# renmengye/rec-attend-public

Measured on AMD Instinct MI355X. Metric: instance-timesteps/sec, full_model forward 512x512 T=16 (whole job; pipelined throughput: 8 batches in flight per GPU, fill and drain of the pipeline inside the timed region; config.lone_batch_* = one sync-bracketed forward), higher is better.
Workload: dtype f32; 1 GPU; cfg2: CVPPP-arch full_model eval forward, 512x512, T=16, B=8 per GPU, y_out+s_out; arch=cvppp, H=512, W=512, T=16, batch_per_gpu=8, global_batch=8, parallelism=batch-sharded x1, no collective, ranks_in_communicator=1, hip_graph=True, tile_tickets=False, batches_in_flight=8, pipeline_slots=4, batches_per_launch=2, input=resident in HBM, output=left in HBM

## Files before the change

include/recattend.h:

```cpp
#ifndef RECATTEND_H_
#define RECATTEND_H_

#include <stddef.h>
#include <stdint.h>

#ifdef __cplusplus
extern "C" {
#endif

#define RA_E_INVALID (-1)
#define RA_E_SHAPE (-2)
#define RA_E_WORKSPACE (-3)
#define RA_E_HUNG_BFS (-12)
#define RA_E_HUNG_PATH (-13)
#define RA_E_HUNG_FLOW (-14)
#define RA_E_HUNG_EQUALIZE (-15)

#define RA_ABI_VERSION 113
int ra_version(void);
const char *ra_last_error_string(void);

int ra_debug_poison_lds(void *stream);
int ra_debug_park_xcd(int xcd, int n_wg, int lds_bytes, int millis, int *resident, void *stream);

#define RA_PLAN_INTS 24
#define RA_PLAN_FAMILY 0
#define RA_PLAN_FORM 1
#define RA_PLAN_CK 2
#define RA_PLAN_NC 3
#define RA_PLAN_WN 4
#define RA_PLAN_GX 5
#define RA_PLAN_GY 6
#define RA_PLAN_KF 7
#define RA_PLAN_TILE_H 8
#define RA_PLAN_TILE_W 9
#define RA_PLAN_TILES_X 10
#define RA_PLAN_TILES_Y 11
#define RA_PLAN_NTILES 12
#define RA_PLAN_GRID 13
#define RA_PLAN_TILES_MIN 14
#define RA_PLAN_TILES_MAX 15
#define RA_PLAN_XCD_MAP 16
#define RA_PLAN_TICKETS 17
#define RA_PLAN_CMID 18
#define RA_PLAN_SLICES 19
#define RA_PLAN_POOL 20
#define RA_PLAN_FAMILY_K1 1
#define RA_PLAN_FAMILY_CONV8 2
#define RA_PLAN_FAMILY_PAIR 3
#define RA_PLAN_FAMILY_SPLIT 4
#define RA_PLAN_FAMILY_WINO 5
#define RA_PLAN_FAMILY_PAIR_WINO 6
#define RA_PLAN_FORM_SWAP 1
#define RA_PLAN_FORM_SUBPIXEL 2
#define RA_PLAN_FORM_BF16 4
#define RA_PLAN_FORM_MOMENTS 8
#define RA_PLAN_FORM_KXK 16
#define RA_PLAN_FORM_PERSIST 32
#define RA_PLAN_FORM_NPACKED 64
#define RA_PLAN_FORM_CACHED 128
#define RA_PLAN_FORM_SPLIT 256
#define RA_PLAN_FORM_PLANE 512
int ra_conv3x3_plan(int C0, int C1, int B, int Hs, int Ws, int upsample, int KF, int Cout, int pool, int has_plane,
                    int bf16_operands, int moments, int store_flags, int *plan);
int ra_conv_pair_plan(int Cin, int B, int Hs, int Ws, int upsampleA, int CoutA, int CoutB, int poolB, int has_plane,
                      int cache_form, int *plan);
int ra_conv_split_plan(int B, int H, int W, int Cin, int Cout, int pool, int has_plane, int *plan);
int ra_conv_wino_plan(int B, int H, int W, int Cin, int Cout, int pool, int *plan);
int ra_conv_pair_wino_plan(int B, int H, int W, int *plan);

int ra_hungarian_f32(const float *weights, int B, int N, int M, float *matching,
                     float *cover_x, float *cover_y);

size_t ra_hungarian_dev_workspace_bytes(int B, int N, int M);
int ra_hungarian_f32_dev(const float *weights, int B, int N, int M, float *matching,
                         float *cover_x, float *cover_y, int *status_dev, void *ws,
                         size_t ws_bytes, void *stream);

#define RA_CONV_TRANSPOSED 1

int ra_conv_cout_padded(int Cout);
size_t ra_conv_packed_floats(int Cin, int Cout);
int ra_conv_pack_weights(const float *w, int Cin_w, int Cout, int Cin, const int *chan_map,
                         int flags, float *out);
size_t ra_conv_packed_floats_k(int KF, int Cin, int Cout);
int ra_conv_pack_weights_k(const float *w, int KF, int Cin_w, int Cout, int Cin, const int *chan_map, int flags,
                           float *out);
int ra_conv_fold_bn(const float *bias, const float *beta, const float *gamma, const float *mean,
                    const float *var, int Cout, float eps, float *scale, float *shift);

int ra_conv3x3_f32(const float *src0, int C0, const float *src1, int C1, int B, int Hs, int Ws,
                   int upsample, const float *wpacked, const float *scale, const float *shift,
                   int Cout, int relu, int pool, const float *plane, int plane_chan, float *y,
                   void *stream);

int ra_convkxk_f32(const float *src0, int C0, const float *src1, int C1, int B, int Hs, int Ws, int upsample,
                   const float *wpacked, int KF, const float *scale, const float *shift, int Cout, int relu, int pool,
                   const float *plane, int plane_chan, float *y, void *stream);

int ra_conv_wide_supported(int Cin, int Cout);
size_t ra_conv_wide_packed_floats(int Cin, int Cout);
int ra_conv_wide_pack_weights(const float *w, int Cin_w, int Cout, int Cin, const int *chan_map, int flags, float *out);
int ra_conv3x3_wide_f32(const float *src0, int C0, const float *src1, int C1, int B, int Hs, int Ws, int upsample,
                        const float *wpacked, const float *scale, const float *shift, int Cout, int relu, int pool,
                        float *y, void *stream);

int ra_fg_head_f32(const float *logits, size_t npix, int nsc, int no, int quantise, float *y_out, float *d_out,
                   const float *x, int D, float *packed, int Cp, float *canvas_plane, void *stream);

int ra_conv3x3_bf16ops_f32(const float *src0, int C0, const float *src1, int C1, int B, int Hs, int Ws,
                           int upsample, const float *wpacked, const float *scale, const float *shift,
                           int Cout, int relu, int pool, const float *plane, int plane_chan, float *y,
                           void *stream);

int ra_conv3x3_bf16_f32(const void *src0, int C0, const void *src1, int C1, int B, int Hs, int Ws, int upsample,
                        const float *wpacked, const float *scale, const float *shift, int Cout, int relu, int pool, void *y,
                        float *part, size_t part_floats, int *nparts, int store_flags, void *stream);
int ra_bn_act_pool_bf16_f32(const void *u, const float *mean, const float *var, const float *gamma, const float *beta, float eps,
                            int relu, int pool, int B, int H, int W, int C, void *y, int flags, void *stream);
int ra_bn_act_pool_bwd_acc_bf16_f32(const void *u, const void *dy, const float *mean, const float *var, const float *gamma,
                                    const float *beta, float eps, int relu, int pool, int B, int H, int W, int C, float *ws,
                                    size_t ws_floats, float *dgamma, float *dbeta, void *du, float *acc_gamma, float *acc_beta,
                                    int flags, void *stream);
int ra_bn_act_pool_bwd_grouped_bf16_f32(const void *u, const void *dy, const void *const *tabs, int G, float eps, int relu, int pool,
                                        int B, int H, int W, int C, float *ws, size_t ws_floats, float *dgamma, float *dbeta,
                                        void *du, int flags, void *stream);
int ra_conv3x3_wgrad_acc_bf16_f32(const void *x, int Cin, int B, int Hs, int Ws, int upsample, const void *du, int Cout, float *ws,
                                  size_t ws_floats, const int *chan_map, int cin_w, int transposed, float *gw, float *gb, int fmt,
                                  void *stream);

size_t ra_conv3x3_moments_part_floats(int Cout);
int ra_conv3x3_moments_f32(const float *src0, int C0, const float *src1, int C1, int B, int Hs, int Ws,
                           int upsample, const float *wpacked, const float *scale, const float *shift,
                           int Cout, int relu, int bf16_operands, float *y, float *part, size_t part_floats,
                           int *nparts, void *stream);
int ra_bn_moments_from_partials_f32(const float *part, int nparts, int C, float *mean, float *var, void *stream);

int ra_conv_pair_supported(int Cin, int CoutA, int CoutB);
int ra_conv_pair_f32(const float *src, int Cin, int B, int Hs, int Ws, int upsampleA,
                     const float *wpA, const float *scaleA, const float *shiftA, int CoutA, int reluA,
                     const float *wpB, const float *scaleB, const float *shiftB, int CoutB, int reluB,
                     int poolB, const float *plane, int plane_chan, float *y, void *stream);

int ra_conv_split_supported(int Cin, int Cout, int pool, int H, int W);
size_t ra_conv_split_packed_halfs(int Cin, int Cout);
int ra_conv_split_pack_weights(const float *w, int Cin, int Cout, unsigned short *out);
int ra_conv_split_pack_weights_dev(const float *w, int Cin, int Cout, int transposed, unsigned short *out, void *stream);
int ra_conv_split_f32(const float *x, int B, int H, int W, int Cin, const unsigned short *wpacked, const float *scale,
                      const float *shift, int Cout, int relu, int pool, float *y, void *stream);
int ra_conv_split_plane_f32(const float *x, int B, int H, int W, int Cin, const float *plane, int plane_chan,
                            const unsigned short *wpacked, const float *scale, const float *shift, int Cout, int relu, int pool,
                            float *y, void *stream);

int ra_conv_wino_supported(int Cin, int Cout, int pool, int H, int W);
size_t ra_conv_wino_packed_floats(int Cin, int Cout);
int ra_conv_wino_pack_weights(const float *w, int Cin, int Cout, float *out);
int ra_conv_wino_f32(const float *x, int B, int H, int W, int Cin, const float *wpacked,
                     const float *scale, const float *shift, int Cout, int relu, int pool, float *y,
                     void *stream);

int ra_conv_pair_wino_supported(int Cin, int CoutA, int CoutB, int poolB, int H, int W);
int ra_conv_pair_wino_f32(const float *x, int B, int H, int W, const float *wpA, const float *scaleA,
                          const float *shiftA, int reluA, const float *wpB_wino, const float *scaleB,
                          const float *shiftB, int reluB, float *y, void *stream);

int ra_conv_first_cache_supported(int Cin, int CoutA, int CoutB, int poolB, int H, int W);
size_t ra_conv_first_cache_floats(int B, int H, int W);
int ra_conv_first_cache_f32(const float *src, int B, int H, int W, const float *wpA, int CoutA,
                            int plane_chan, float *cache, void *stream);
int ra_conv_pair_fill_cache_f32(const float *src, const float *plane, int plane_chan, int B, int H,
                                int W, const float *wpA, const float *scaleA, const float *shiftA,
                                int reluA, const float *wpB, const float *scaleB,
                                const float *shiftB, int CoutB, int reluB, float *cache, float *y,
                                void *stream);
int ra_conv_pair_fill_cache_rider_f32(const float *src, const float *plane, int plane_chan, int B, int H, int W,
                                      const float *wpA, const float *scaleA, const float *shiftA, int reluA,
                                      const float *wpB, const float *scaleB, const float *shiftB, int CoutB,
                                      int reluB, float *cache, float *y, float *fill_dst, size_t fill_floats,
                                      float fill_value, void *stream);
int ra_conv_pair_cached_f32(const float *cache, const float *plane, int plane_chan, int B, int H,
                            int W, const float *wpA, const float *scaleA, const float *shiftA,
                            int reluA, const float *wpB, const float *scaleB, const float *shiftB,
                            int CoutB, int reluB, float *y, void *stream);

typedef struct ra_ctrl_desc {
  int G;
  int Cf;
  int hid;
  int iters;
  int n_gmlp;
  int n_cmlp;
  int mlp_dim;
  int H, W;
  int Fh, Fw;
  int squash;
  int fixed_var;
  int dynamic_var;
  int fixed_gamma;
} ra_ctrl_desc;

size_t ra_ctrl_packed_floats(const ra_ctrl_desc *d);
int ra_ctrl_pack_weights(const ra_ctrl_desc *d, const float *const *lstm_w,
                         const float *const *gmlp_w, const float *const *cmlp_w, float *out);

#define RA_ATTN_STRIDE 16
int ra_controller_f32(const ra_ctrl_desc *d, const float *feat , const float *wpacked,
                      int B, float *h_last , float *ctrl_out ,
                      float *glimpse_maps ,
                      float *attn , void *stream);

int ra_ctrl_split_supported(const ra_ctrl_desc *d);
size_t ra_ctrl_split_packed_floats(const ra_ctrl_desc *d);
size_t ra_ctrl_split_workspace_bytes(const ra_ctrl_desc *d, int B);
int ra_ctrl_split_pack_weights(const ra_ctrl_desc *d, const float *const *lstm_w,
                               const float *const *gmlp_w, const float *const *cmlp_w, float *out);
int ra_controller_split_f32(const ra_ctrl_desc *d, const float *feat, const float *wpacked, int B,
                            float *h_last, float *ctrl_out, float *glimpse_maps, float *attn,
                            void *ws, size_t ws_bytes, int *status_dev, void *stream);
int ra_ctrl_batch_group_images(const ra_ctrl_desc *d, int B);
int ra_ctrl_batch_supported(const ra_ctrl_desc *d);
// ... 272 lines not shown
```

rec-attend-public_amd/csrc/ra_conv_split.hip:

```cpp
#include <cstring>

#include "ra_common.h"

namespace ra {
namespace csplit {

typedef float f32x4 __attribute__((ext_vector_type(4)));
typedef float f32x2 __attribute__((ext_vector_type(2)));
typedef short s16x8 __attribute__((ext_vector_type(8)));
typedef __bf16 bf16x8 __attribute__((ext_vector_type(8)));
typedef unsigned u32x2 __attribute__((ext_vector_type(2)));
typedef unsigned u32x4 __attribute__((ext_vector_type(4)));

constexpr int TW = 16;
constexpr int WSX = TW + 2;
constexpr int WSP = 20;
constexpr int tile_rows(int cin) { return (cin >= 64 || cin == 24) ? 8 : 16; }
constexpr int rec_stride(int cin) { return cin == 24 ? 80 : 2 * cin + 16; }
constexpr int k_blocks(int cin) { return (9 * (cin / 8) + 3) / 4; }

struct SArgs {
  const float *x;
  const unsigned short *wp;
  const float *scale, *shift;
  float *y;
  int B, H, W, Cout, relu;
  int bytes_x, bytes_y;
  unsigned *tickets;
  const float *plane;
  int plane_chan, bytes_p;
};

template <int CIN, int NB>
struct Geo {
  static constexpr int TH = tile_rows(CIN), WSY = TH + 2;
  static constexpr int GPW = TH / 4;
  static constexpr int NBLK = k_blocks(CIN);
  static constexpr int RS = rec_stride(CIN);
  static constexpr int PLANE = WSY * WSP * RS;
  static constexpr int WBYTES = NBLK * 3 * NB * 1024;
  static constexpr int LDS = 3 * PLANE + WBYTES;
  static constexpr int OCC = 2 * (LDS + 64) <= 160 * 1024 ? 2 : 1;
};

__device__ inline unsigned pk_bf16(float lo, float hi) {
  typedef __bf16 bf16x2c __attribute__((ext_vector_type(2)));
  return __builtin_bit_cast(unsigned, __builtin_convertvector(f32x2{lo, hi}, bf16x2c));
}
__device__ inline void split3_pair(float a, float b, unsigned &H, unsigned &M, unsigned &L) {
  H = pk_bf16(a, b);
  float ra = a - __builtin_bit_cast(float, H << 16), rb = b - __builtin_bit_cast(float, H & 0xffff0000u);
  M = pk_bf16(ra, rb);
  ra -= __builtin_bit_cast(float, M << 16);
  rb -= __builtin_bit_cast(float, M & 0xffff0000u);
  L = pk_bf16(ra, rb);
}

#ifdef RA_PROBES
__device__ long long *ra_probes_buf;
#define RA_PS_DECL long long ps_acc[8] = {0, 0, 0, 0, 0, 0, 0, 0}, ps_t = (long long)__builtin_readcyclecounter(), ps_t0 = (long long)wall_clock64()
#define RA_PS_AT(k)                                                \
  do {                                                             \
    __builtin_amdgcn_sched_barrier(0);                             \
    const long long n_ = (long long)__builtin_readcyclecounter();  \
    ps_acc[k] += n_ - ps_t;                                        \
    ps_t = n_;                                                     \
    __builtin_amdgcn_sched_barrier(0);                             \
  } while (0)
#define RA_PS_END                                                                    \
  do {                                                                               \
    if (threadIdx.x == 0 && ra_probes_buf) {                                         \
      ps_acc[7] = (long long)wall_clock64() - ps_t0;                                 \
      for (int k_ = 0; k_ < 8; ++k_) ra_probes_buf[((size_t)blockIdx.y * gridDim.x + blockIdx.x) * 8 + k_] = ps_acc[k_]; \
    }                                                                                \
  } while (0)
#else
#define RA_PS_DECL
#define RA_PS_AT(k)
#define RA_PS_END
#endif
template <int CIN, int POOL, int NB, bool PL = false>
__global__ __launch_bounds__(256, (Geo<CIN, NB>::OCC)) void conv_split_kernel(const SArgs a, int tiles_x, int tiles_y, int ntiles) {
  using G = Geo<CIN, NB>;
  constexpr int RS = G::RS, PLANE = G::PLANE, NBLK = G::NBLK, C4 = CIN / 4, TH = G::TH, WSY = G::WSY, GPW = G::GPW;
  constexpr int NITEMS = WSY * WSX * C4, NIT = (NITEMS + 255) / 256;
  extern __shared__ __attribute__((aligned(16))) unsigned char lds[];
  unsigned char *tin = lds;
  unsigned char *wl = lds + 3 * PLANE;
  const int tid = threadIdx.x, lane = tid & 63;
  RA_PS_DECL;
  __shared__ unsigned tk_sh[2];
  TicketWalk tk;
  const bool dyn = a.tickets != nullptr;
  if (dyn) tk.issue(a.tickets + blockIdx.y * kTicketSlotWords, ntiles);
  const int wave = __builtin_amdgcn_readfirstlane(tid >> 6);
  const int m = lane & 15, kb = lane >> 4;
  const int slice = blockIdx.y;

  const int qy = m >> 3, qx = (m >> 2) & 1, dy = (m >> 1) & 1, dx = m & 1;
  const int lane_pix = ((2 * qy + dy) * WSP + 2 * qx + dx) * RS;
  int toff[NBLK];
#pragma unroll
  for (int b = 0; b < NBLK; ++b) {
    constexpr int OPT = CIN / 8;
    const int o = 4 * b + kb;
    int tap = o / OPT;
    const int ch = 8 * (o % OPT);
    tap = tap < 9 ? tap : 8;
    toff[b] = ((tap / 3) * WSP + tap % 3) * RS + 2 * ch;
  }
  const int woff = (kb * 16 + m) * 16;
  float sc[NB], sh[NB];
#pragma unroll
  for (int nb = 0; nb < NB; ++nb) {
    sc[nb] = a.scale[16 * (NB * slice + nb) + m];
    sh[nb] = a.shift[16 * (NB * slice + nb) + m];
  }
  const float lo = a.relu ? 0.f : -__builtin_inff();
  const int Ho = a.H / POOL, Wo = a.W / POOL;
  const __amdgpu_buffer_rsrc_t rx = __builtin_amdgcn_make_buffer_rsrc(const_cast<float *>(a.x), 0, a.bytes_x, 0x00020000);
  const __amdgpu_buffer_rsrc_t ry = __builtin_amdgcn_make_buffer_rsrc(a.y, 0, a.bytes_y, 0x00020000);
  const int per = tiles_x * tiles_y;

  int it_off[NIT], it_r[NIT], it_c[NIT], it_lds[NIT], it_pl[PL ? NIT : 1];
#pragma unroll
  for (int i = 0; i < NIT; ++i) {
    const int e = tid + 256 * i;
    const int c4 = e % C4, pix = e / C4;
    it_r[i] = pix / WSX;
    it_c[i] = pix - it_r[i] * WSX;
    it_off[i] = ((it_r[i] * a.W + it_c[i]) * CIN + 4 * c4) * 4;
    it_lds[i] = (it_r[i] * WSP + it_c[i]) * RS + 8 * c4;
    if (e >= NITEMS) it_r[i] = -(1 << 20);
    if constexpr (PL) it_pl[i] = (c4 == (a.plane_chan >> 2)) ? (it_r[i] * a.W + it_c[i]) * 4 : -1;
  }
  const __amdgpu_buffer_rsrc_t rp = __builtin_amdgcn_make_buffer_rsrc(const_cast<float *>(PL ? a.plane : a.x), 0, PL ? a.bytes_p : 0, 0x00020000);
  const int pl_lane = a.plane_chan & 3;
  f32x4 preA[NIT], preB[NIT];
  float plA[PL ? NIT : 1], plB[PL ? NIT : 1];
  auto fetch = [&](int T, f32x4(&pre)[NIT], float(&ppl)[PL ? NIT : 1]) {
    const int fb = T / per, fr = T - fb * per;
    const int fy0 = (fr / tiles_x) * TH - 1, fx0 = (fr % tiles_x) * TW - 1;
    const int base = ((fb * a.H + fy0) * a.W + fx0) * CIN * 4;
#pragma unroll
    for (int i = 0; i < NIT; ++i) {
      const int Y = fy0 + it_r[i], X = fx0 + it_c[i];
      const bool ok = (Y >= 0) & (Y < a.H) & (X >= 0) & (X < a.W);
      pre[i] = __builtin_bit_cast(f32x4, __builtin_amdgcn_raw_buffer_load_b128(rx, ok ? base + it_off[i] : 0x7fffffff, 0, 0));
    }
    if constexpr (PL) {
      const int pbase = ((fb * a.H + fy0) * a.W + fx0) * 4;
#pragma unroll
      for (int i = 0; i < NIT; ++i) {
        const int Y = fy0 + it_r[i], X = fx0 + it_c[i];
        const bool ok = (it_pl[i] >= 0) & (Y >= 0) & (Y < a.H) & (X >= 0) & (X < a.W);
        ppl[i] = __builtin_bit_cast(float, __builtin_amdgcn_raw_buffer_load_b32(rp, ok ? pbase + it_pl[i] : 0x7fffffff, 0, 0));
      }
    }
  };

  constexpr int NWQ = G::WBYTES / 16, NWI = (NWQ + 255) / 256;
  u32x4 wtmp[NWI];
  {
    const u32x4 *src = reinterpret_cast<const u32x4 *>(reinterpret_cast<const unsigned char *>(a.wp) + (size_t)slice * G::WBYTES);
#pragma unroll
    for (int i = 0; i < NWI; ++i) {
      const int e = tid + 256 * i;
      wtmp[i] = src[e < NWQ ? e : NWQ - 1];
    }
  }
  int tile = blockIdx.x, tnext = 0;
  const int gstep = (int)gridDim.x;
  if (dyn) {
    tk.begin(tk_sh);
    tile = tk.cur >= 0 ? tk.cur : ntiles;
  }
  if (tile < ntiles) fetch(tile, preA, plA);
  if (!dyn && tile + gstep < ntiles) fetch(tile + gstep, preB, plB);
#pragma unroll
  for (int i = 0; i < NWI; ++i) {
    const int e = tid + 256 * i;
    if (e < NWQ) reinterpret_cast<u32x4 *>(wl)[e] = wtmp[i];
  }
  RA_PS_AT(0);

  auto stage = [&](f32x4(&pre)[NIT], float(&ppl)[PL ? NIT : 1]) {
    __syncthreads();
    RA_PS_AT(1);
#pragma unroll
    for (int i = 0; i < NIT; ++i) {
      f32x4 v = pre[i];
      if constexpr (PL) {
        if (it_pl[i] >= 0) {
          v.x = pl_lane == 0 ? ppl[i] : v.x;
          v.y = pl_lane == 1 ? ppl[i] : v.y;
          v.z = pl_lane == 2 ? ppl[i] : v.z;
          v.w = pl_lane == 3 ? ppl[i] : v.w;
        }
      }
      unsigned H0, M0, L0, H1, M1, L1;
      split3_pair(v.x, v.y, H0, M0, L0);
      split3_pair(v.z, v.w, H1, M1, L1);
      if (it_r[i] >= 0) {
        unsigned char *rec = tin + it_lds[i];
        *reinterpret_cast<u32x2 *>(rec) = u32x2{H0, H1};
        *reinterpret_cast<u32x2 *>(rec + PLANE) = u32x2{M0, M1};
        *reinterpret_cast<u32x2 *>(rec + 2 * PLANE) = u32x2{L0, L1};
      }
    }
    RA_PS_AT(2);
    if (dyn) tk.publish(tk_sh);
    __syncthreads();
    RA_PS_AT(3);
  };

  auto compute = [&](int T) {
    const int b = T / per, trem = T - b * per;
    const int ty = trem / tiles_x, tx = trem - ty * tiles_x;
    f32x4 acc[GPW][NB];
#pragma unroll
    for (int g = 0; g < GPW; ++g)
#pragma unroll
      for (int nb = 0; nb < NB; ++nb) acc[g][nb] = f32x4{0.f, 0.f, 0.f, 0.f};
    const int grow = GPW == 4 ? wave : wave >> 1, gx0 = GPW == 4 ? 0 : 2 * (wave & 1);
    const int wave_pix = (4 * grow * WSP + 4 * gx0) * RS + lane_pix;
    constexpr int PA[6] = {1, 0, 2, 0, 1, 0}, PB[6] = {1, 2, 0, 1, 0, 0};
#pragma unroll
    for (int blk = 0; blk < NBLK; ++blk) {
      s16x8 wv[3][NB];
#pragma unroll
      for (int pc = 0; pc < 3; ++pc)
#pragma unroll
        for (int nb = 0; nb < NB; ++nb) wv[pc][nb] = *reinterpret_cast<const s16x8 *>(wl + ((blk * 3 + pc) * NB + nb) * 1024 + woff);
#pragma unroll
      for (int g = 0; g < GPW; ++g) {
        s16x8 av[3];
#pragma unroll
        for (int pc = 0; pc < 3; ++pc) av[pc] = *reinterpret_cast<const s16x8 *>(tin + pc * PLANE + wave_pix + 4 * g * RS + toff[blk]);
#pragma unroll
        for (int t = 0; t < 6; ++t)
#pragma unroll
          for (int nb = 0; nb < NB; ++nb)
            acc[g][nb] = __builtin_amdgcn_mfma_f32_16x16x32_bf16(__builtin_bit_cast(bf16x8, av[PA[t]]), __builtin_bit_cast(bf16x8, wv[PB[t]][nb]),
                                                                 acc[g][nb], 0, 0, 0);
      }
    }
    RA_PS_AT(4);
    const int wy = kb >> 1, wx = kb & 1;
#pragma unroll
    for (int g = 0; g < GPW; ++g)
#pragma unroll
      for (int nb = 0; nb < NB; ++nb) {
        const int co = 16 * (NB * slice + nb) + m;
        const f32x4 v = acc[g][nb] * sc[nb] + sh[nb];
        if constexpr (POOL == 2) {
          const float o = fmaxf(fmaxf(fmaxf(v[0], v[1]), fmaxf(v[2], v[3])), lo);
          const int oy = ty * (TH / 2) + 2 * grow + wy, ox = tx * (TW / 2) + 2 * (gx0 + g) + wx;
          if ((ox < Wo) & (oy < Ho))
            __builtin_amdgcn_raw_buffer_store_b32(__builtin_bit_cast(unsigned, o), ry, (((b * Ho + oy) * Wo + ox) * a.Cout + co) * 4, 0, 0);
        } else {
#pragma unroll
          for (int r = 0; r < 4; ++r) {
            const int oy = ty * TH + 4 * grow + 2 * wy + (r >> 1), ox = tx * TW + 4 * (gx0 + g) + 2 * wx + (r & 1);
            if ((ox < Wo) & (oy < Ho))
              __builtin_amdgcn_raw_buffer_store_b32(__builtin_bit_cast(unsigned, fmaxf(v[r], lo)), ry,
                                                    (((b * Ho + oy) * Wo + ox) * a.Cout + co) * 4, 0, 0);
          }
        }
      }
    RA_PS_AT(5);
  };

  if (dyn) {
    for (; tile < ntiles; tile = tnext) {
      stage(preA, plA);
      tk.read_next(tk_sh);
      tk.request();
      tk.step();
      tnext = tk.cur >= 0 ? tk.cur : ntiles;
      if (tnext < ntiles) fetch(tnext, preA, plA);
      compute(tile);
    }
  } else {
    for (; tile < ntiles; tile += 2 * gstep) {
      stage(preA, plA);
      if (tile + 2 * gstep < ntiles) fetch(tile + 2 * gstep, preA, plA);
      compute(tile);
      if (tile + gstep >= ntiles) break;
      stage(preB, plB);
      if (tile + 3 * gstep < ntiles) fetch(tile + 3 * gstep, preB, plB);
      compute(tile + gstep);
    }
  }
  RA_PS_END;
}

inline int cu_count() {
  static int cus = 0;
  if (!cus) {
    hipDeviceProp_t prop;
    int dev = 0;
    cus = 256;
    if (hipGetDevice(&dev) == hipSuccess && hipGetDeviceProperties(&prop, dev) == hipSuccess) cus = prop.multiProcessorCount;
  }
  return cus;
}

template <int CIN, int POOL, int NB, bool PL = false>
int launch(const SArgs &a, hipStream_t st, int *plan) {
  auto kern = conv_split_kernel<CIN, POOL, NB, PL>;
  constexpr int lds = Geo<CIN, NB>::LDS;
  const int tiles_x = (a.W + TW - 1) / TW, tiles_y = (a.H + Geo<CIN, NB>::TH - 1) / Geo<CIN, NB>::TH, ntiles = tiles_x * tiles_y * a.B, slices = a.Cout / (16 * NB);
  int gx = Geo<CIN, NB>::OCC * cu_count() / slices;
  if (gx < 1) gx = 1;
  if (gx > ntiles) gx = ntiles;
  SArgs a2 = a;
  const bool draws = ntiles >= kTicketMinTilesPerWg * gx;
  if (plan) {
    plan[RA_PLAN_FAMILY] = RA_PLAN_FAMILY_SPLIT, plan[RA_PLAN_FORM] = PL ? RA_PLAN_FORM_PLANE : 0;
    plan[RA_PLAN_CK] = CIN, plan[RA_PLAN_NC] = NB, plan[RA_PLAN_KF] = 3, plan[RA_PLAN_POOL] = POOL, plan[RA_PLAN_SLICES] = slices;
    plan[RA_PLAN_TILE_H] = Geo<CIN, NB>::TH, plan[RA_PLAN_TILE_W] = TW, plan[RA_PLAN_TILES_X] = tiles_x, plan[RA_PLAN_TILES_Y] = tiles_y;
    plan[RA_PLAN_TICKETS] = draws ? 1 : 0;
    plan_walk(plan, ntiles, gx, 0);
    return 0;
  }
  static const MaxDynamicLds lds_limit(kern, lds);
  a2.tickets = draws ? take_ticket_slots(slices, gx) : nullptr;
  hipLaunchKernelGGL(kern, dim3(gx, slices), dim3(256), lds, st, a2, tiles_x, tiles_y, ntiles);
  return launch_status("ra_conv_split_f32");
}

inline unsigned short bf16_rne_host(float v) {
  unsigned u;
  memcpy(&u, &v, 4);
  u += 0x7fffu + ((u >> 16) & 1u);
  return (unsigned short)(u >> 16);
}
inline float bf16_to_float_host(unsigned short h) {
  const unsigned u = (unsigned)h << 16;
  float f;
  memcpy(&f, &u, 4);
  return f;
}

}
}

using namespace ra;

extern "C" int ra_conv_split_supported(int Cin, int Cout, int pool, int H, int W) {
  return (Cin == 16 || Cin == 24 || Cin == 32 || Cin == 64) && Cout > 0 && Cout % 16 == 0 && (pool == 1 || pool == 2) && H > 0 && W > 0 &&
         H % 4 == 0 && W % 4 == 0;
}

extern "C" size_t ra_conv_split_packed_halfs(int Cin, int Cout) {
  if (!(Cin == 16 || Cin == 24 || Cin == 32 || Cin == 64) || Cout <= 0 || Cout % 16) return 0;
  return (size_t)(Cout / 16) * csplit::k_blocks(Cin) * 3 * 512;
}

namespace ra {
namespace csplit {
__host__ __device__ inline void slot_of(size_t e, int Cin, int Cout, int nblk, int nbw, int &pc, int &tap, int &ci, int &co) {
  const int j = (int)(e & 7), nn = (int)((e >> 3) & 15), kb = (int)((e >> 7) & 3);
  size_t r = e >> 9;
  const int nb = (int)(r % nbw);
  r /= nbw;
  pc = (int)(r % 3);
  r /= 3;
  const int b = (int)(r % nblk), s = (int)(r / nblk);
  const int o = 4 * b + kb, opt = Cin / 8;
  tap = o / opt;
  ci = 8 * (o % opt) + j;
  co = 16 * (nbw * s + nb) + nn;
}
__host__ __device__ inline float filter_at(const float *w, int Cin, int Cout, int transposed, int tap, int ci, int co) {
  if (tap >= 9) return 0.f;
  return transposed ? w[((size_t)(8 - tap) * Cout + co) * Cin + ci] : w[((size_t)tap * Cin + ci) * Cout + co];
}
__global__ __launch_bounds__(256) void pack_split_kernel(const float *w, int Cin, int Cout, int transposed, int nblk, int nbw, size_t n,
                                                         unsigned short *out) {
  const size_t e = (size_t)blockIdx.x * 256 + threadIdx.x;
  if (e >= n) return;
  int pc, tap, ci, co;
  slot_of(e, Cin, Cout, nblk, nbw, pc, tap, ci, co);
  float v = filter_at(w, Cin, Cout, transposed, tap, ci, co);
  unsigned short h = 0;
  for (int k = 0; k <= pc; ++k) {
    unsigned u = __builtin_bit_cast(unsigned, v);
    u += 0x7fffu + ((u >> 16) & 1u);
    h = (unsigned short)(u >> 16);
    v -= __builtin_bit_cast(float, (unsigned)h << 16);
  }
  out[e] = h;
}
}
}

extern "C" int ra_conv_split_pack_weights_dev(const float *w, int Cin, int Cout, int transposed, unsigned short *out, void *stream) {
  const size_t n = ra_conv_split_packed_halfs(Cin, Cout);
  if (!w || !out || !n) return fail(RA_E_SHAPE, "ra_conv_split_pack_weights_dev: Cin=%d Cout=%d", Cin, Cout);
  const int nblk = csplit::k_blocks(Cin), nbw = (Cout % 32 == 0 && Cin < 64) ? 2 : 1;
  hipLaunchKernelGGL(csplit::pack_split_kernel, dim3((unsigned)((n + 255) / 256)), dim3(256), 0, as_stream(stream), w, Cin, Cout,
                     transposed ? 1 : 0, nblk, nbw, n, out);
  return launch_status("ra_conv_split_pack_weights_dev");
}

extern "C" int ra_conv_split_pack_weights(const float *w, int Cin, int Cout, unsigned short *out) {
  const size_t n = ra_conv_split_packed_halfs(Cin, Cout);
  if (!w || !out || !n) return fail(RA_E_SHAPE, "ra_conv_split_pack_weights: Cin=%d Cout=%d", Cin, Cout);
  const int nblk = csplit::k_blocks(Cin), nbw = (Cout % 32 == 0 && Cin < 64) ? 2 : 1;
  for (size_t e = 0; e < n; ++e) {
    int pc, tap, ci, co;
    csplit::slot_of(e, Cin, Cout, nblk, nbw, pc, tap, ci, co);
    float v = csplit::filter_at(w, Cin, Cout, 0, tap, ci, co);
    unsigned short h = 0;
    for (int k = 0; k <= pc; ++k) {
      h = csplit::bf16_rne_host(v);
      v -= csplit::bf16_to_float_host(h);
    }
    out[e] = h;
  }
  return 0;
}

namespace ra {
namespace csplit {
int run(const float *x, int B, int H, int W, int Cin, const float *plane, int plane_chan, const unsigned short *wpacked, const float *scale,
        const float *shift, int Cout, int relu, int pool, float *y, void *stream, const char *who, int *plan = nullptr) {
  if ((!plan && (!x || !wpacked || !scale || !shift || !y)) || B <= 0) return fail(RA_E_INVALID, "%s: bad argument", who);
  if (!ra_conv_split_supported(Cin, Cout, pool, H, W))
    return fail(RA_E_SHAPE, "%s: Cin=%d Cout=%d pool=%d %dx%d", who, Cin, Cout, pool, H, W);
  if (plane && (plane_chan < 0 || plane_chan >= Cin)) return fail(RA_E_INVALID, "%s: plane_chan %d outside [0, %d)", who, plane_chan, Cin);
  const size_t bx = (size_t)B * H * W * Cin * 4, by = (size_t)B * (H / pool) * (W / pool) * Cout * 4;
  if (bx >= (1ull << 31) || by >= (1ull << 31)) return fail(RA_E_SHAPE, "%s: a tensor exceeds 2 GiB", who);
  SArgs a{};
  a.x = x;
  a.wp = wpacked;
  a.scale = scale;
  a.shift = shift;
  a.y = y;
  a.B = B;
  a.H = H;
  a.W = W;
  a.Cout = Cout;
  a.relu = relu;
  a.bytes_x = (int)bx;
  a.bytes_y = (int)by;
  a.plane = plane;
  a.plane_chan = plane ? plane_chan : 0;
  a.bytes_p = (int)((size_t)B * H * W * 4);
  hipStream_t st = as_stream(stream);
  const bool two = Cout % 32 == 0 && Cin < 64;
#define RA_CS(CIN_)                                                                                             \
  if (Cin == CIN_) {                                                                                            \
    if (plane) {                                                                                                \
      if (two) return pool == 2 ? launch<CIN_, 2, 2, true>(a, st, plan) : launch<CIN_, 1, 2, true>(a, st, plan);            \
      return pool == 2 ? launch<CIN_, 2, 1, true>(a, st, plan) : launch<CIN_, 1, 1, true>(a, st, plan);                     \
    }                                                                                                           \
    if (two) return pool == 2 ? launch<CIN_, 2, 2>(a, st, plan) : launch<CIN_, 1, 2>(a, st, plan);                          \
    return pool == 2 ? launch<CIN_, 2, 1>(a, st, plan) : launch<CIN_, 1, 1>(a, st, plan);                                   \
  }
  RA_CS(16)
  RA_CS(24)
  RA_CS(32)
#undef RA_CS
  if (plane) return fail(RA_E_SHAPE, "%s: the plane form is built for Cin 16 / 24 / 32", who);
  return pool == 2 ? launch<64, 2, 1>(a, st, plan) : launch<64, 1, 1>(a, st, plan);
}
}
}

extern "C" int ra_conv_split_f32(const float *x, int B, int H, int W, int Cin, const unsigned short *wpacked, const float *scale,
                                 const float *shift, int Cout, int relu, int pool, float *y, void *stream) {
  return csplit::run(x, B, H, W, Cin, nullptr, 0, wpacked, scale, shift, Cout, relu, pool, y, stream, "ra_conv_split_f32");
}

extern "C" int ra_conv_split_plane_f32(const float *x, int B, int H, int W, int Cin, const float *plane, int plane_chan,
                                       const unsigned short *wpacked, const float *scale, const float *shift, int Cout, int relu, int pool,
                                       float *y, void *stream) {
  if (!plane) return fail(RA_E_INVALID, "ra_conv_split_plane_f32: null plane");
  return csplit::run(x, B, H, W, Cin, plane, plane_chan, wpacked, scale, shift, Cout, relu, pool, y, stream, "ra_conv_split_plane_f32");
}

extern "C" int ra_conv_split_plan(int B, int H, int W, int Cin, int Cout, int pool, int has_plane, int *plan) {
  if (!plan) return fail(RA_E_INVALID, "ra_conv_split_plan: bad argument");
  for (int i = 0; i < RA_PLAN_INTS; ++i) plan[i] = 0;
  if (!plan_have_device()) return fail(RA_E_INVALID, "ra_conv_split_plan: the grid is the device's CU count: no device");
  static float mark;
  return csplit::run(nullptr, B, H, W, Cin, has_plane ? &mark : nullptr, 0, nullptr, nullptr, nullptr, Cout, 0, pool, nullptr, nullptr,
                     "ra_conv_split_plan", plan);
}
```

rec-attend-public_amd/ra_ops.py:

```python
import ctypes as C

import numpy as np
import torch

import ra_native as rn
from ra_native import check, ptr

BN_EPS = 1e-3


def _need_cuda(*ts):
  for t in ts:
    if t is not None and not t.is_cuda:
      raise rn.RecAttendError('recattend kernels need CUDA (HIP) tensors; got a CPU tensor. '
                              'There is no CPU fallback.')
    if t is not None and (t.dtype != torch.float32 or not t.is_contiguous()):
      raise rn.RecAttendError('recattend kernels need contiguous float32 tensors')


def _np32(a):
  if isinstance(a, torch.Tensor):
    a = a.detach().cpu().numpy()
  return np.ascontiguousarray(a, dtype=np.float32)

# ... 160 lines not shown
    return torch.empty(shape, dtype=torch.float32, device=src.device)
  if checked_for and tuple(out.shape) != shape:
    raise rn.RecAttendError('%s: out of shape %r, expected %r' % (checked_for, tuple(out.shape), shape))
  return out


def conv3x3(src0, wp, scale, shift, cout, relu=True, pool=1, src1=None, upsample=False,
            out=None, plane=None, plane_chan=-1, bf16=False):
  _need_cuda(src0, src1, wp, scale, shift, out)
  B, Hs, Ws, C0 = src0.shape
  C1 = 0 if src1 is None else src1.shape[3]
  out = _conv_out(src0, cout, pool, upsample, out)
  fn = rn.lib().ra_conv3x3_bf16ops_f32 if bf16 else rn.lib().ra_conv3x3_f32
  check(fn(ptr(src0), C0, ptr(src1), C1, B, Hs, Ws, int(upsample), ptr(wp), ptr(scale), ptr(shift), int(cout),
           int(relu), int(pool), ptr(plane), int(plane_chan), ptr(out), rn.stream_ptr()),
        'ra_conv3x3_bf16ops_f32' if bf16 else 'ra_conv3x3_f32')
  return out


_PLAN_FAMILIES = {v: k[len('RA_PLAN_FAMILY_'):].lower() for k, v in rn.CONSTANTS.items() if k.startswith('RA_PLAN_FAMILY_')}
_PLAN_FORMS = sorted((v, k[len('RA_PLAN_FORM_'):].lower()) for k, v in rn.CONSTANTS.items() if k.startswith('RA_PLAN_FORM_'))
_PLAN_FIELDS = sorted((v, k[len('RA_PLAN_'):].lower()) for k, v in rn.CONSTANTS.items()
                      if k.startswith('RA_PLAN_') and not k.startswith(('RA_PLAN_FAMILY_', 'RA_PLAN_FORM_')) and k != 'RA_PLAN_INTS')


def plan_dict(rec):
  out = {field: rec[i] for i, field in _PLAN_FIELDS}
  out['family'] = _PLAN_FAMILIES[rec[rn.RA_PLAN_FAMILY]]
  out['form'] = tuple(sorted(n for bit, n in _PLAN_FORMS if rec[rn.RA_PLAN_FORM] & bit))
  return out


def _plan(name, *args):
  rec = (C.c_int * rn.RA_PLAN_INTS)()
  check(getattr(rn.lib(), name)(*([int(a) for a in args] + [rec])), name)
  return plan_dict(rec)


def conv3x3_plan(c0, c1, B, Hs, Ws, cout, pool=1, upsample=False, ksize=3, plane=False, bf16=False, moments=False, store_flags=0):
  return _plan('ra_conv3x3_plan', c0, c1, B, Hs, Ws, bool(upsample), ksize, cout, pool, bool(plane), bool(bf16), bool(moments), store_flags)


def conv_pair_plan(cin, B, Hs, Ws, couta, coutb, poolB=2, upsampleA=False, plane=False, cache_form=0):
  return _plan('ra_conv_pair_plan', cin, B, Hs, Ws, bool(upsampleA), couta, coutb, poolB, bool(plane), cache_form)


def conv_split_plan(B, H, W, cin, cout, pool=1, plane=False):
  return _plan('ra_conv_split_plan', B, H, W, cin, cout, pool, bool(plane))


def conv_wino_plan(B, H, W, cin, cout, pool=1):
  return _plan('ra_conv_wino_plan', B, H, W, cin, cout, pool)


def conv_pair_wino_plan(B, H, W):
  return _plan('ra_conv_pair_wino_plan', B, H, W)


def conv2d_fused(src0, wp, scale, shift, cout, ksize, relu=True, pool=1, src1=None, upsample=False, out=None, plane=None,
                 plane_chan=-1):
  if cout > 128:
    if ksize != 3 or plane is not None:
      raise rn.RecAttendError('wide layers (Cout = %d > 128) are built for 3x3 filters without a canvas plane' % cout)
    return conv_wide(src0, wp, scale, shift, cout, relu=relu, pool=pool, src1=src1, upsample=upsample, out=out)
  if ksize == 3:
    return conv3x3(src0, wp, scale, shift, cout, relu=relu, pool=pool, src1=src1, upsample=upsample, out=out, plane=plane,
                   plane_chan=plane_chan)
  _need_cuda(src0, src1, wp, scale, shift, out)
  B, Hs, Ws, C0 = src0.shape
  C1 = 0 if src1 is None else src1.shape[3]
  out = _conv_out(src0, cout, pool, upsample, out)
  check(rn.lib().ra_convkxk_f32(ptr(src0), C0, ptr(src1), C1, B, Hs, Ws, int(upsample), ptr(wp), int(ksize), ptr(scale),
                                ptr(shift), int(cout), int(relu), int(pool), ptr(plane), int(plane_chan), ptr(out),
                                rn.stream_ptr()), 'ra_convkxk_f32')
  return out


def conv_wide_supported(cin, cout):
  return bool(rn.lib().ra_conv_wide_supported(int(cin), int(cout)))


def pack_wide_weights(w, cin_kernel=None, chan_map=None, transposed=False):
  w = _np32(w)
  if w.ndim != 4 or tuple(w.shape[:2]) != (3, 3):
    raise rn.RecAttendError('filter of shape %r: wide layers are built for 3x3 filters only' % (w.shape,))
  cin_w, cout, cin, chan_map, flags = _filter_channels(w, cin_kernel, chan_map, transposed)
  n = rn.lib().ra_conv_wide_packed_floats(cin, cout)
  if n == 0:
    raise rn.RecAttendError('unsupported wide conv shape Cin=%d Cout=%d (Cin %% 4, <= 1024; Cout 129 .. 512, %% 16)' % (cin, cout))
  out = np.empty(n, dtype=np.float32)
  cm = _chan_map_i32(chan_map, cin)
  check(rn.lib().ra_conv_wide_pack_weights(ptr(w), cin_w, cout, cin, ptr(cm), flags, ptr(out)), 'ra_conv_wide_pack_weights')
  return out


def conv_wide(src0, wp, scale, shift, cout, relu=True, pool=1, src1=None, upsample=False, out=None):
  _need_cuda(src0, src1, wp, scale, shift, out)
  B, Hs, Ws, C0 = src0.shape
  C1 = 0 if src1 is None else src1.shape[3]
  if src1 is not None and tuple(src1.shape[:3]) != (B, Hs, Ws):
    raise rn.RecAttendError('conv_wide: sources of %r and %r' % (tuple(src0.shape), tuple(src1.shape)))
  n = rn.lib().ra_conv_wide_packed_floats(C0 + C1, int(cout))
  if n == 0 or wp.numel() != n or scale.numel() < cout or shift.numel() < cout:
    raise rn.RecAttendError('conv_wide: unsupported shape Cin=%d Cout=%d, or weights not packed for it' % (C0 + C1, cout))
  out = _conv_out(src0, cout, pool, upsample, out, checked_for='conv_wide')
  check(rn.lib().ra_conv3x3_wide_f32(ptr(src0), C0, ptr(src1), C1, B, Hs, Ws, int(upsample), ptr(wp), ptr(scale), ptr(shift),
                                     int(cout), int(relu), int(pool), ptr(out), rn.stream_ptr()), 'ra_conv3x3_wide_f32')
  return out


def fg_head(logits, nsc, no, quantise=False, y_out=None, d_out=None, x=None, packed=None, canvas_plane=None):
  _need_cuda(logits, y_out, d_out, x, packed, canvas_plane)
  B, H, W, C = logits.shape
  if C != nsc + no:
    raise rn.RecAttendError('fg_head: %d channels for nsc %d + no %d' % (C, nsc, no))
  npix = B * H * W
  f = lambda c: torch.empty((B, H, W, c), dtype=torch.float32, device=logits.device)
  if y_out is None:
    y_out = f(nsc)
  if d_out is None and no:
    d_out = f(no)
  if y_out.numel() != npix * nsc or (no and d_out.numel() != npix * no):
    raise rn.RecAttendError('fg_head: destination sizes')
  D = Cp = 0
  if packed is not None:
    if x is None or x.numel() % npix or packed.numel() % npix:
      raise rn.RecAttendError('fg_head: the packed destination needs x [B,H,W,D]')
    D, Cp = x.numel() // npix, packed.numel() // npix
    if canvas_plane is not None and canvas_plane.numel() != npix:
      raise rn.RecAttendError('fg_head: canvas plane size')
  check(rn.lib().ra_fg_head_f32(ptr(logits), npix, int(nsc), int(no), int(bool(quantise)), ptr(y_out), ptr(d_out if no else None),
                                ptr(x if packed is not None else None), D, ptr(packed), Cp,
                                ptr(canvas_plane if packed is not None else None), rn.stream_ptr()), 'ra_fg_head_f32')
  return y_out, (d_out if no else None)


def conv_wino_supported(cin, cout, pool, H, W):
  return bool(rn.lib().ra_conv_wino_supported(int(cin), int(cout), int(pool), int(H), int(W)))


def pack_wino_weights(w):
  w = _np32(w)
  cin, cout = w.shape[2], w.shape[3]
  n = rn.lib().ra_conv_wino_packed_floats(cin, cout)
  if w.shape[0] != 3 or w.shape[1] != 3 or n == 0:
    raise rn.RecAttendError('unsupported Winograd conv shape %r' % (w.shape,))
  out = np.empty(n, dtype=np.float32)
  check(rn.lib().ra_conv_wino_pack_weights(ptr(w), cin, cout, ptr(out)), 'ra_conv_wino_pack_weights')
  return out


def conv_split_supported(cin, cout, pool, H, W):
  return bool(rn.lib().ra_conv_split_supported(int(cin), int(cout), int(pool), int(H), int(W)))


def pack_split_weights(w, cin_kernel=None, chan_map=None):
  w = _np32(w)
  if cin_kernel is not None or chan_map is not None:
    ck = int(cin_kernel if cin_kernel is not None else len(chan_map))
    cm = list(chan_map) if chan_map is not None else list(range(w.shape[2])) + [-1] * (ck - w.shape[2])
    wk = np.zeros((3, 3, ck, w.shape[3]), np.float32)
    for c, m_ in enumerate(cm[:ck]):
      if m_ >= 0:
        wk[:, :, c, :] = w[:, :, m_, :]
    w = wk
  cin, cout = w.shape[2], w.shape[3]
  n = rn.lib().ra_conv_split_packed_halfs(cin, cout)
  if w.shape[0] != 3 or w.shape[1] != 3 or n == 0:
    raise rn.RecAttendError('unsupported split-precision conv shape %r' % (w.shape,))
  out = np.empty(n, dtype=np.int16)
  check(rn.lib().ra_conv_split_pack_weights(ptr(w), cin, cout, ptr(out)), 'ra_conv_split_pack_weights')
  return out.view(np.float32)


def pack_split_weights_dev(w, cin, cout, transposed=False):
  _need_cuda(w)
  n = rn.lib().ra_conv_split_packed_halfs(int(cin), int(cout))
  if n == 0 or w.numel() != 9 * cin * cout:
    raise rn.RecAttendError('unsupported split-precision conv shape Cin=%d Cout=%d' % (cin, cout))
  out = torch.empty(n // 2, dtype=torch.float32, device=w.device)
  check(rn.lib().ra_conv_split_pack_weights_dev(ptr(w.contiguous()), int(cin), int(cout), int(bool(transposed)), ptr(out),
                                                rn.stream_ptr()), 'ra_conv_split_pack_weights_dev')
  return out


def conv_split(x, wp, scale, shift, cout, relu=True, pool=1, out=None, plane=None, plane_chan=-1):
  _need_cuda(x, wp, scale, shift, out, plane)
  B, H, W, cin = x.shape
  out = _conv_out(x, cout, pool, out=out)
  if plane is not None:
    check(rn.lib().ra_conv_split_plane_f32(ptr(x), B, H, W, cin, ptr(plane), int(plane_chan), ptr(wp), ptr(scale), ptr(shift), int(cout),
                                           int(relu), int(pool), ptr(out), rn.stream_ptr()), 'ra_conv_split_plane_f32')
    return out
  check(rn.lib().ra_conv_split_f32(ptr(x), B, H, W, cin, ptr(wp), ptr(scale), ptr(shift), int(cout), int(relu), int(pool),
                                   ptr(out), rn.stream_ptr()), 'ra_conv_split_f32')
  return out


def conv_wino(x, wp, scale, shift, cout, relu=True, pool=1, out=None):
  _need_cuda(x, wp, scale, shift, out)
  B, H, W, cin = x.shape
  out = _conv_out(x, cout, pool, out=out)
  check(rn.lib().ra_conv_wino_f32(ptr(x), B, H, W, cin, ptr(wp), ptr(scale), ptr(shift), int(cout), int(relu), int(pool),
                                  ptr(out), rn.stream_ptr()), 'ra_conv_wino_f32')
  return out


def conv_pair_wino_supported(cin, cout_a, cout_b, pool_b, H, W):
  return bool(rn.lib().ra_conv_pair_wino_supported(int(cin), int(cout_a), int(cout_b), int(pool_b), int(H), int(W)))


def conv_pair_wino(x, wpA, scA, shA, wpB_wino, scB, shB, reluA=True, reluB=True, out=None):
  _need_cuda(x, wpA, scA, shA, wpB_wino, scB, shB, out)
  B, H, W, _ = x.shape
  out = _conv_out(x, 16, 2, out=out)
  check(rn.lib().ra_conv_pair_wino_f32(ptr(x), B, H, W, ptr(wpA), ptr(scA), ptr(shA), int(reluA), ptr(wpB_wino), ptr(scB),
                                       ptr(shB), int(reluB), ptr(out), rn.stream_ptr()), 'ra_conv_pair_wino_f32')
  return out


def poison_lds():
  check(rn.lib().ra_debug_poison_lds(rn.stream_ptr()), 'ra_debug_poison_lds')


def park_xcd(xcd, n_wg, lds_bytes=100 * 1024, millis=100, resident=None, stream=None):
  check(rn.lib().ra_debug_park_xcd(int(xcd), int(n_wg), int(lds_bytes), int(millis), ptr(resident) if resident is not None else None,
                                   rn.stream_ptr() if stream is None else stream.cuda_stream), 'ra_debug_park_xcd')


def conv_pair_supported(cin, cout_a, cout_b):
  return bool(rn.lib().ra_conv_pair_supported(int(cin), int(cout_a), int(cout_b)))


def conv_pair(src, wpA, scA, shA, coutA, wpB, scB, shB, coutB, poolB=1, upsampleA=False,
              reluA=True, reluB=True, out=None, plane=None, plane_chan=-1):
  _need_cuda(src, wpA, scA, shA, wpB, scB, shB, out)
  B, Hs, Ws, C0 = src.shape
  out = _conv_out(src, coutB, poolB, upsampleA, out)
  check(rn.lib().ra_conv_pair_f32(ptr(src), C0, B, Hs, Ws, int(upsampleA), ptr(wpA), ptr(scA),
                                  ptr(shA), int(coutA), int(reluA), ptr(wpB), ptr(scB), ptr(shB),
                                  int(coutB), int(reluB), int(poolB), ptr(plane), int(plane_chan),
                                  ptr(out), rn.stream_ptr()),
        'ra_conv_pair_f32')
  return out


def first_cache_supported(cin, cout_a, cout_b, pool_b, H, W):
  return bool(rn.lib().ra_conv_first_cache_supported(int(cin), int(cout_a), int(cout_b), int(pool_b), int(H), int(W)))


def first_cache_alloc(B, H, W, device):
  return torch.zeros((rn.lib().ra_conv_first_cache_floats(B, H, W),), dtype=torch.float32, device=device)


def first_cache(img, wpA, cout_a, plane_chan, cache):
  _need_cuda(img, wpA, cache)
  B, H, W, C = img.shape
  assert C == 4
  check(rn.lib().ra_conv_first_cache_f32(ptr(img), B, H, W, ptr(wpA), int(cout_a), int(plane_chan), ptr(cache),
                                         rn.stream_ptr()), 'ra_conv_first_cache_f32')


def fill_rider_ok(t):
  return t.is_contiguous() and t.data_ptr() % 16 == 0 and t.numel() % 4 == 0 and t.numel() * 4 < (1 << 31)


def conv_pair_fill_cache(img, plane, plane_chan, wpA, scA, shA, wpB, scB, shB, coutB, cache, out, reluA=True, reluB=True,
                         fill=None, fill_value=0.0):
  _need_cuda(img, plane, wpA, scA, shA, wpB, scB, shB, cache, out, fill)
  B, H, W = plane.shape
  if fill is not None and not fill_rider_ok(fill):
    raise rn.RecAttendError('conv_pair_fill_cache: the rider fill needs a contiguous, 16-byte aligned tensor of 4k floats < 2 GiB')
  check(rn.lib().ra_conv_pair_fill_cache_rider_f32(ptr(img), ptr(plane), int(plane_chan), B, H, W, ptr(wpA), ptr(scA),
                                                   ptr(shA), int(reluA), ptr(wpB), ptr(scB), ptr(shB), int(coutB),
                                                   int(reluB), ptr(cache), ptr(out), ptr(fill),
                                                   0 if fill is None else fill.numel(), C.c_float(fill_value),
                                                   rn.stream_ptr()),
        'ra_conv_pair_fill_cache_rider_f32')
  return out


def conv_pair_cached(cache, plane, plane_chan, wpA, scA, shA, wpB, scB, shB, coutB, out, reluA=True, reluB=True):
  _need_cuda(cache, plane, wpA, scA, shA, wpB, scB, shB, out)
  B, H, W = plane.shape
  check(rn.lib().ra_conv_pair_cached_f32(ptr(cache), ptr(plane), int(plane_chan), B, H, W, ptr(wpA), ptr(scA),
                                         ptr(shA), int(reluA), ptr(wpB), ptr(scB), ptr(shB), int(coutB),
                                         int(reluB), ptr(out), rn.stream_ptr()), 'ra_conv_pair_cached_f32')
  return out


def controller(desc, feat, wp, h_last, ctrl_out, gmaps, attn):
  _need_cuda(feat, wp, h_last, ctrl_out, gmaps, attn)
  B = feat.shape[0]
  check(rn.lib().ra_controller_f32(C.byref(desc), ptr(feat), ptr(wp), B, ptr(h_last),
                                   ptr(ctrl_out), ptr(gmaps), ptr(attn), rn.stream_ptr()),
        'ra_controller_f32')


def extract_direct(img, chan0, attn, Fh, Fw, Cp, use_gamma, patch, canvas=None, canvas_chan=-1):
  _need_cuda(img, attn, patch, canvas)
  B, H, W, Ci = img.shape
  check(rn.lib().ra_extract_direct_f32(ptr(img), Ci, chan0, ptr(canvas), int(canvas_chan), ptr(attn),
                                       B, H, W, Fh, Fw, Cp, int(use_gamma), ptr(patch),
                                       rn.stream_ptr()), 'ra_extract_direct_f32')


# ... 503 lines not shown
```

Measured before the change: 57430 instance-timesteps/s.

## Re-stride split-conv LDS tiles and duplicate Cin=24 octets to avoid bank conflicts

Changes the per-pixel LDS record stride of the split-precision conv (32/96/160 bytes by Cin) and, for Cin=24, stores each channel octet twice at swizzled slots so A-operand reads from different lane quadrants land in distinct banks. Occupancy is now set explicitly (2 workgroups per CU only for small Cin with NB=1), and a static_assert guards the LDS budget. A host-callable layout query is added for testing. The cost is extra LDS stores for Cin=24 and possibly lower occupancy for some configurations that previously fit two workgroups.

```diff
diff --git a/include/recattend.h b/include/recattend.h
--- a/include/recattend.h
+++ b/include/recattend.h
@@ -66,6 +66,7 @@
 int ra_conv_pair_plan(int Cin, int B, int Hs, int Ws, int upsampleA, int CoutA, int CoutB, int poolB, int has_plane,
                       int cache_form, int *plan);
 int ra_conv_split_plan(int B, int H, int W, int Cin, int Cout, int pool, int has_plane, int *plan);
+int ra_conv_split_lds_layout(int Cin, int NB, int block, int *offsets, int *lds_bytes, int *occ);
 int ra_conv_wino_plan(int B, int H, int W, int Cin, int Cout, int pool, int *plan);
 int ra_conv_pair_wino_plan(int B, int H, int W, int *plan);
 
diff --git a/rec-attend-public_amd/csrc/ra_conv_split.hip b/rec-attend-public_amd/csrc/ra_conv_split.hip
--- a/rec-attend-public_amd/csrc/ra_conv_split.hip
+++ b/rec-attend-public_amd/csrc/ra_conv_split.hip
@@ -16,8 +16,19 @@
 constexpr int WSX = TW + 2;
 constexpr int WSP = 20;
 constexpr int tile_rows(int cin) { return (cin >= 64 || cin == 24) ? 8 : 16; }
-constexpr int rec_stride(int cin) { return cin == 24 ? 80 : 2 * cin + 16; }
+constexpr int rec_stride(int cin) { return cin == 16 ? 32 : cin == 64 ? 160 : 96; }
+__host__ __device__ constexpr int octet_slot(int cin, int j, int h) { return cin == 24 ? j + 3 * ((j ^ h) & 1) : j; }
+constexpr int octet_copies(int cin) { return cin == 24 ? 2 : 1; }
 constexpr int k_blocks(int cin) { return (9 * (cin / 8) + 3) / 4; }
+__host__ __device__ constexpr int a_operand_offset(int cin, int lane, int blk) {
+  const int m = lane & 15, kb = lane >> 4, qy = m >> 3, qx = (m >> 2) & 1, dy = (m >> 1) & 1, dx = m & 1;
+  const int opt = cin / 8, o = 4 * blk + kb, tap = o / opt < 9 ? o / opt : 8;
+  return ((2 * qy + dy + tap / 3) * WSP + 2 * qx + dx + tap % 3) * rec_stride(cin) + 16 * octet_slot(cin, o % opt, qy ^ qx);
+}
+__host__ __device__ constexpr int stage_offset(int cin, int r, int c, int c4, int copy) {
+  return (r * WSP + c) * rec_stride(cin) + 16 * octet_slot(cin, c4 >> 1, copy) + 8 * (c4 & 1);
+}
+constexpr int wg_per_cu(int cin, int nb) { return cin <= 24 && nb == 1 ? 2 : 1; }
 
 struct SArgs {
   const float *x;
@@ -40,7 +51,8 @@
   static constexpr int PLANE = WSY * WSP * RS;
   static constexpr int WBYTES = NBLK * 3 * NB * 1024;
   static constexpr int LDS = 3 * PLANE + WBYTES;
-  static constexpr int OCC = 2 * (LDS + 64) <= 160 * 1024 ? 2 : 1;
+  static constexpr int OCC = wg_per_cu(CIN, NB);
+  static_assert(OCC * (LDS + 64) <= 160 * 1024, "the workgroups of a CU share 160 KiB of LDS");
 };
 
 __device__ inline unsigned pk_bf16(float lo, float hi) {
@@ -97,18 +109,9 @@
   const int m = lane & 15, kb = lane >> 4;
   const int slice = blockIdx.y;
 
-  const int qy = m >> 3, qx = (m >> 2) & 1, dy = (m >> 1) & 1, dx = m & 1;
-  const int lane_pix = ((2 * qy + dy) * WSP + 2 * qx + dx) * RS;
   int toff[NBLK];
 #pragma unroll
-  for (int b = 0; b < NBLK; ++b) {
-    constexpr int OPT = CIN / 8;
-    const int o = 4 * b + kb;
-    int tap = o / OPT;
-    const int ch = 8 * (o % OPT);
-    tap = tap < 9 ? tap : 8;
-    toff[b] = ((tap / 3) * WSP + tap % 3) * RS + 2 * ch;
-  }
+  for (int b = 0; b < NBLK; ++b) toff[b] = a_operand_offset(CIN, lane, b);
   const int woff = (kb * 16 + m) * 16;
   float sc[NB], sh[NB];
 #pragma unroll
@@ -122,7 +125,8 @@
   const __amdgpu_buffer_rsrc_t ry = __builtin_amdgcn_make_buffer_rsrc(a.y, 0, a.bytes_y, 0x00020000);
   const int per = tiles_x * tiles_y;
 
-  int it_off[NIT], it_r[NIT], it_c[NIT], it_lds[NIT], it_pl[PL ? NIT : 1];
+  constexpr int COPIES = octet_copies(CIN);
+  int it_off[NIT], it_r[NIT], it_c[NIT], it_lds[NIT], it_lds2[COPIES == 2 ? NIT : 1], it_pl[PL ? NIT : 1];
 #pragma unroll
   for (int i = 0; i < NIT; ++i) {
     const int e = tid + 256 * i;
@@ -130,7 +134,8 @@
     it_r[i] = pix / WSX;
     it_c[i] = pix - it_r[i] * WSX;
     it_off[i] = ((it_r[i] * a.W + it_c[i]) * CIN + 4 * c4) * 4;
-    it_lds[i] = (it_r[i] * WSP + it_c[i]) * RS + 8 * c4;
+    it_lds[i] = stage_offset(CIN, it_r[i], it_c[i], c4, 0);
+    if constexpr (COPIES == 2) it_lds2[i] = stage_offset(CIN, it_r[i], it_c[i], c4, 1);
     if (e >= NITEMS) it_r[i] = -(1 << 20);
     if constexpr (PL) it_pl[i] = (c4 == (a.plane_chan >> 2)) ? (it_r[i] * a.W + it_c[i]) * 4 : -1;
   }
@@ -206,6 +211,12 @@
         *reinterpret_cast<u32x2 *>(rec) = u32x2{H0, H1};
         *reinterpret_cast<u32x2 *>(rec + PLANE) = u32x2{M0, M1};
         *reinterpret_cast<u32x2 *>(rec + 2 * PLANE) = u32x2{L0, L1};
+        if constexpr (COPIES == 2) {
+          rec = tin + it_lds2[i];
+          *reinterpret_cast<u32x2 *>(rec) = u32x2{H0, H1};
+          *reinterpret_cast<u32x2 *>(rec + PLANE) = u32x2{M0, M1};
+          *reinterpret_cast<u32x2 *>(rec + 2 * PLANE) = u32x2{L0, L1};
+        }
       }
     }
     RA_PS_AT(2);
@@ -223,7 +234,7 @@
 #pragma unroll
       for (int nb = 0; nb < NB; ++nb) acc[g][nb] = f32x4{0.f, 0.f, 0.f, 0.f};
     const int grow = GPW == 4 ? wave : wave >> 1, gx0 = GPW == 4 ? 0 : 2 * (wave & 1);
-    const int wave_pix = (4 * grow * WSP + 4 * gx0) * RS + lane_pix;
+    const int wave_pix = (4 * grow * WSP + 4 * gx0) * RS;
     constexpr int PA[6] = {1, 0, 2, 0, 1, 0}, PB[6] = {1, 2, 0, 1, 0, 0};
 #pragma unroll
     for (int blk = 0; blk < NBLK; ++blk) {
@@ -482,6 +493,18 @@
   return csplit::run(x, B, H, W, Cin, plane, plane_chan, wpacked, scale, shift, Cout, relu, pool, y, stream, "ra_conv_split_plane_f32");
 }
 
+extern "C" int ra_conv_split_lds_layout(int Cin, int NB, int block, int *offsets, int *lds_bytes, int *occ) {
+  const bool form = (Cin == 16 || Cin == 24 || Cin == 32 || Cin == 64) && (NB == 1 || (NB == 2 && Cin < 64));
+  if (!offsets || !lds_bytes || !occ || !form || block < 0 || block >= csplit::k_blocks(Cin))
+    return fail(RA_E_SHAPE, "ra_conv_split_lds_layout: Cin=%d NB=%d block=%d", Cin, NB, block);
+  for (int lane = 0; lane < 64; ++lane) offsets[lane] = csplit::a_operand_offset(Cin, lane, block);
+#define RA_CS(CIN_, NB_) \
+  if (Cin == CIN_ && NB == NB_) *lds_bytes = csplit::Geo<CIN_, NB_>::LDS, *occ = csplit::Geo<CIN_, NB_>::OCC;
+  RA_CS(16, 1) RA_CS(16, 2) RA_CS(24, 1) RA_CS(24, 2) RA_CS(32, 1) RA_CS(32, 2) RA_CS(64, 1)
+#undef RA_CS
+  return 0;
+}
+
 extern "C" int ra_conv_split_plan(int B, int H, int W, int Cin, int Cout, int pool, int has_plane, int *plan) {
   if (!plan) return fail(RA_E_INVALID, "ra_conv_split_plan: bad argument");
   for (int i = 0; i < RA_PLAN_INTS; ++i) plan[i] = 0;
diff --git a/rec-attend-public_amd/ra_ops.py b/rec-attend-public_amd/ra_ops.py
--- a/rec-attend-public_amd/ra_ops.py
+++ b/rec-attend-public_amd/ra_ops.py
@@ -336,6 +336,12 @@
 
 def conv_split_supported(cin, cout, pool, H, W):
   return bool(rn.lib().ra_conv_split_supported(int(cin), int(cout), int(pool), int(H), int(W)))
+
+
+def conv_split_lds_layout(cin, nb, block):
+  offs, lds, occ = (C.c_int * 64)(), C.c_int(), C.c_int()
+  check(rn.lib().ra_conv_split_lds_layout(int(cin), int(nb), int(block), offs, C.byref(lds), C.byref(occ)), 'ra_conv_split_lds_layout')
+  return list(offs), lds.value, occ.value
 
 
 def pack_split_weights(w, cin_kernel=None, chan_map=None):
```

Measured after the change: 55880 instance-timesteps/s. -2.7%, worse.
